# aoschu/esn-ofdm-mimo

Measured on AMD Instinct MI355X. Metric: OFDM symbols/s through the ESN detector (4x8 TDL-B, N=128, N_res=512; train+predict+detect), higher is better.
Workload: dtype f16 operands / f32 accumulate

## Files before the change

### esn_ofdm_mimo_amd/csrc/esn_recur_skew16_impl.h

```cpp
#pragma once
#include "esn_recur_mfma_impl.h"

namespace esn {

constexpr int S16_NKK = 17;
constexpr int S16_NKH = 8;
constexpr int S16_MP = 512;

template <typename TR, int NOISE, bool IO32 = false>
__global__ __launch_bounds__(512) void recur_skew16_kernel(RecurParams p) {
    extern __shared__ __attribute__((aligned(16))) char zf[];
    constexpr int NW = 8, BT = 128, NOWN = 8, NKK = S16_NKK, NKH = S16_NKH;
    constexpr int NTHREADS = NW * 64;
    constexpr int TILE_B = NKK * 1024;
    ESN_STAMP(t_entry)
    const int tid = threadIdx.x;
    const int lane = tid & 63;
    const int wave = __builtin_amdgcn_readfirstlane(tid >> 6);
    const Geometry& g = p.g;
    const int n_res = p.n_res, n_in = p.n_in, n_out = p.n_out;
    const int kin_p = g.kfb - g.kin;
    const int kfb_p = round_up(n_out, 4);
    const int out_rows = p.S - p.transient;

    const int tile = xcd_remap(blockIdx.x, p.n_tiles);
    const int slot0 = tile * BT;
    const int grp0 = slot_group(p, slot0);
    if (grp0 >= p.n_groups) return;
    const int wset = slot_wset(p, slot0);

    int* tab_fr = reinterpret_cast<int*>(zf + (size_t)NOWN * TILE_B);
    uint32_t* tab_key = reinterpret_cast<uint32_t*>(tab_fr + BT);
    float2* tab_in = reinterpret_cast<float2*>(tab_key + BT);
    float2* tab_un = tab_in + NOWN * kin_p;
    char* in_slots = reinterpret_cast<char*>(tab_un + NOWN * 16);
    int* tab_off = reinterpret_cast<int*>(in_slots + (size_t)NOWN * 2048);
    uint32_t* tab_ks = reinterpret_cast<uint32_t*>(tab_off + BT);
    int* tab_grp = reinterpret_cast<int*>(in_slots);
    const int lkin = __builtin_ctz(kin_p);
    for (int i = tid; i < BT; i += NTHREADS) {
        int gtmp;
        const int fr = slot_frame(p, slot0 + i, gtmp);
        tab_fr[i] = fr;
        tab_grp[i] = gtmp;
        tab_key[i] = mix32((uint32_t)p.seed ^ (((uint32_t)fr + p.frame_off) * 0x9E3779B9U));
    }
    {
        constexpr int CHUNKS = NOWN * TILE_B / 16;
        static_assert(CHUNKS % NTHREADS == 0, "whole passes");
#pragma unroll
        for (int i = 0; i < CHUNKS / NTHREADS; ++i)
            *reinterpret_cast<u32x4*>(zf + (size_t)(i * NTHREADS + tid) * 16) = u32x4{0u, 0u, 0u, 0u};
    }
    __syncthreads();
    for (int i = tid; i < NOWN * kin_p; i += NTHREADS) {
        const int c16 = i >> lkin, c = i & (kin_p - 1);
        const int cg = tab_grp[c16 * 16];
        float2 v = make_float2(0.f, 0.f);
        if (cg < p.n_groups && c < n_in) {
            v.x = p.in_scale ? (float)p.in_scale[(size_t)cg * n_in + c] : 1.f;
            v.y = p.in_shift ? (float)p.in_shift[(size_t)cg * n_in + c] : 0.f;
        }
        tab_in[i] = v;
    }
    for (int i = tid; i < NOWN * 16; i += NTHREADS) {
        const int c16 = i / 16, o = i % 16;
        const int cg = tab_grp[c16 * 16];
        float2 v = make_float2(1.f, 0.f);
        if (cg < p.n_groups && o < n_out) {
            if (p.t_scale) v.x = (float)(1.0 / p.t_scale[(size_t)cg * n_out + o]);
            if (p.t_shift) v.y = (float)p.t_shift[(size_t)cg * n_out + o];
        }
        tab_un[i] = v;
    }
#define S16_INLINE __attribute__((always_inline))
    if (p.x0) {
        for (int i = tid; i < BT * 2 * NKH * 4; i += NTHREADS) {
            const int f = i & (BT - 1), kq = i >> 7, kk = kq >> 2, q = kq & 3;
            const bool live = tab_fr[f] >= 0;
            const double* xr = p.x0 + (size_t)(live ? tab_grp[f] : 0) * n_res;
            uint32_t w[4];
#pragma unroll
            for (int t = 0; t < 2; ++t) {
                const int k = 32 * kk + 16 * t + 4 * q;
                float v[4];
#pragma unroll
                for (int e = 0; e < 4; ++e) v[e] = (live && k + e < n_res) ? (float)xr[k + e] : 0.f;
                w[2 * t] = TR::pack2(v[0], v[1]);
                w[2 * t + 1] = TR::pack2(v[2], v[3]);
            }
            *reinterpret_cast<u32x4*>(zf + ((size_t)((f >> 4) * NKK + kk) * 64 + q * 16 + (f & 15)) * 16) = u32x4{w[0], w[1], w[2], w[3]};
        }
    }
    if (p.y0) {
        for (int i = tid; i < BT * 2; i += NTHREADS) {
            const int f = i & (BT - 1), o0 = 4 * (i >> 7);
            const bool live = tab_fr[f] >= 0;
            const double* yr = p.y0 + (size_t)(live ? tab_grp[f] : 0) * n_out;
            float v[4];
#pragma unroll
            for (int e = 0; e < 4; ++e) v[e] = (live && o0 + e < n_out) ? (float)yr[o0 + e] : 0.f;
            const int pos = g.kfb - S16_MP + o0;
            if (o0 < kfb_p)
                TR::store4(zf + ((size_t)((f >> 4) * NKK + 16) * 64 + (pos >> 3) * 16 + (f & 15)) * 16 + 2 * (pos & 7),
                           v[0], v[1], v[2], v[3]);
        }
    }
    __syncthreads();

    const int own_grp = __builtin_amdgcn_readfirstlane(slot_group(p, slot0 + wave * 16));
    const bool has_ro = own_grp < p.n_groups;
    float wo_inv = 1.f;
    if (has_ro)
        wo_inv = *reinterpret_cast<const float*>(reinterpret_cast<const char*>(p.packed_wout)
                                                 + (size_t)own_grp * p.wout_stride + p.wo16_off + (size_t)NKK * 1024);
    const uint32_t in_stride = (uint32_t)(p.T_in * n_in);
    for (int e = tid; e < BT * kin_p; e += NTHREADS) {
        const int f = e >> lkin, ci = e & (kin_p - 1);
        const int fr = tab_fr[f];
        float v = 0.f;
        if (fr >= 0 && ci < n_in) {
            const int row = p.in_row_off;
            const double raw = (row < p.T_in) ? (double)in_ptr<IO32>(p)[(size_t)fr * in_stride + (size_t)row * n_in + ci] : 0.0;
            const float2 ss = tab_in[(f >> 4) * kin_p + ci];
            v = fmaf((float)raw, ss.x, ss.y);
        }
        TR::store1(zf + ((size_t)((f >> 4) * NKK + 16) * 64 + (ci >> 3) * 16 + (f & 15)) * 16 + 2 * (ci & 7), v);
    }

    const float noise = (float)p.noise;
    const float n_c1 = noise * (1.0f / 256.0f), n_c0 = noise * (0.5f / 256.0f - 0.5f);
    f32x4 yacc = {0.f, 0.f, 0.f, 0.f};
    const int lane16 = lane * 16;
    constexpr int OOB = 0x7ffffff0;

    auto finish_readout = [&](int orow, bool write_fb) S16_INLINE {
        int ln_ro = lane;
        asm volatile("" : "+v"(ln_ro));
        const int ofc = ln_ro & 15, oq = ln_ro >> 4;
        if (!has_ro) return;
        const int of = wave * 16 + ofc;
        f32x4 y = yacc;
        const int o0 = 4 * oq;
        const int fr = tab_fr[of];
        const float4* un4 = reinterpret_cast<const float4*>(tab_un + wave * 16 + o0);
        const float4 u01 = un4[0], u23 = un4[1];
#pragma unroll
        for (int j = 0; j < 4; ++j) y[j] += __shfl_xor(y[j], 32);
        y *= wo_inv;
        if (o0 < kfb_p) {
            if (write_fb) {
                const int pos = g.kfb - S16_MP + o0;
                TR::store4(zf + ((size_t)(wave * NKK + 16) * 64 + (pos >> 3) * 16 + ofc) * 16 + 2 * (pos & 7),
                           y[0], y[1], y[2], y[3]);
            }
            if (IO32 && orow >= 0 && fr >= 0) {
                float* yo = p.Y32 + ((size_t)fr * out_rows + orow) * n_out;
                if ((n_out & 3) == 0) {
                    *reinterpret_cast<float4*>(yo + o0) =
                        make_float4((y[0] - u01.y) * u01.x, (y[1] - u01.w) * u01.z, (y[2] - u23.y) * u23.x, (y[3] - u23.w) * u23.z);
                } else {
                    const float2* un = tab_un + wave * 16 + o0;
#pragma unroll
                    for (int j = 0; j < 4; ++j)
                        if (o0 + j < n_out) yo[o0 + j] = (y[j] - un[j].y) * un[j].x;
                }
            } else if (!IO32 && orow >= 0 && fr >= 0) {
                double* yo = p.Y + ((size_t)fr * out_rows + orow) * n_out;
                if ((n_out & 3) == 0) {
                    typedef double f64x2s __attribute__((ext_vector_type(2)));
                    *reinterpret_cast<f64x2s*>(yo + o0) =
                        f64x2s{(double)((y[0] - u01.y) * u01.x), (double)((y[1] - u01.w) * u01.z)};
                    *reinterpret_cast<f64x2s*>(yo + o0 + 2) =
                        f64x2s{(double)((y[2] - u23.y) * u23.x), (double)((y[3] - u23.w) * u23.z)};
                } else {
                    const float2* un = tab_un + wave * 16 + o0;
#pragma unroll
                    for (int j = 0; j < 4; ++j)
                        if (o0 + j < n_out) yo[o0 + j] = (double)((y[j] - un[j].y) * un[j].x);
                }
            }
        }
        yacc = f32x4{0.f, 0.f, 0.f, 0.f};
    };

    const int lag = wave >= NW / 2 ? 1 : 0;
    f32x4 acc[4][8];
    u32x4 abuf[2][4], b[4], ra[4];
    auto zero_acc = [&]() S16_INLINE {
#pragma unroll
        for (int m = 0; m < 4; ++m)
#pragma unroll
            for (int n = 0; n < 8; ++n) acc[m][n] = f32x4{0.f, 0.f, 0.f, 0.f};
    };
    const __amdgpu_buffer_rsrc_t w_rsrc = __builtin_amdgcn_make_buffer_rsrc(
        const_cast<char*>(reinterpret_cast<const char*>(p.packed_w) + (size_t)wset * p.wset_stride + p.w16_off), 0,
        S16_MP * NKK * 64, 0x00020000);
    const int w_frag0 = wave * NKK * 4;
    auto loadA = [&](u32x4 (&a)[4], int kk) S16_INLINE {
        const bool live = kk < NKK;
        const int voff = live ? lane16 : OOB;
#pragma unroll
        for (int m = 0; m < 4; ++m)
            a[m] = __builtin_bit_cast(u32x4, __builtin_amdgcn_raw_buffer_load_b128(
                w_rsrc, voff, live ? (w_frag0 + kk * 4 + m) * 1024 : 0, 0));
    };
    const __amdgpu_buffer_rsrc_t wo_rsrc = __builtin_amdgcn_make_buffer_rsrc(
        const_cast<char*>(reinterpret_cast<const char*>(p.packed_wout)
                          + (size_t)(has_ro ? own_grp : 0) * p.wout_stride + p.wo16_off),
        0, NKK * 1024 + 16, 0x00020000);
    auto load_ra = [&](int j, int kk, bool on) S16_INLINE {
        on = on && kk < 2 * NKH;
        const int voff = on ? lane16 : OOB;
        ra[2 * j] = __builtin_bit_cast(u32x4, __builtin_amdgcn_raw_buffer_load_b128(wo_rsrc, voff, on ? kk * 1024 : 0, 0));
        ra[2 * j + 1] = __builtin_bit_cast(u32x4, __builtin_amdgcn_raw_buffer_load_b128(wo_rsrc, voff, on ? (kk ^ 8) * 1024 : 0, 0));
    };
    auto ro_prefetch = [&](int kk0, bool on) S16_INLINE { load_ra(0, kk0, on); load_ra(1, kk0 + 1, on); };
    typedef const __attribute__((address_space(3))) u32x4* lds_frag_t;
    auto gemm_half = [&](int kk0, auto ro_tag, bool ro_on) S16_INLINE {
        constexpr bool RO = decltype(ro_tag)::value;
        const int voff_ro = ro_on ? lane16 : OOB;
        int ln = lane;
        asm volatile("" : "+v"(ln));
        const uint32_t zb = (uint32_t)(uintptr_t)zf + (uint32_t)(ln << 4);
        uint32_t bp0 = zb + (uint32_t)kk0 * 1024;
        uint32_t bp1 = bp0 + 4 * TILE_B;
#pragma unroll
        for (int n = 0; n < 4; ++n) b[n] = *reinterpret_cast<lds_frag_t>((uintptr_t)(bp0 + n * TILE_B));
        uint32_t rp = zb + (uint32_t)(wave * TILE_B) + (uint32_t)kk0 * 1024;
        uint32_t xp = zb + (uint32_t)(wave * TILE_B) + (uint32_t)(kk0 ^ 8) * 1024;
        int sA = (w_frag0 + (kk0 + 2) * 4) * 1024;
        int sR = (kk0 + 2) * 1024;
        auto trip = [&](int i, auto tail_tag) S16_INLINE {
            constexpr bool TAIL = decltype(tail_tag)::value;
#pragma unroll
            for (int j = 0; j < 2; ++j) {
                const int kk = kk0 + i + j;
                u32x4 rb0, rbx;
#pragma unroll
                for (int n = 0; n < 8; ++n) {
#pragma unroll
                    for (int m = 0; m < 4; ++m) {
                        TR::mma16(acc[m][n], abuf[j][m], b[n & 3]);
                        const int u = n * 4 + m;
                        if (RO) {
                            if (u == 0) rb0 = *reinterpret_cast<lds_frag_t>((uintptr_t)(rp + j * 1024));
                            if (u == 1) rbx = *reinterpret_cast<lds_frag_t>((uintptr_t)(xp + j * 1024));
                            if (u == 8) {
                                TR::mma16(yacc, ra[2 * j], rb0);
                                if (!TAIL)
                                    ra[2 * j] = __builtin_bit_cast(u32x4, __builtin_amdgcn_raw_buffer_load_b128(
                                        wo_rsrc, voff_ro, sR + j * 1024, 0));
                            }
                            if (u == 10) {
                                TR::mma16(yacc, ra[2 * j + 1], rbx);
                                if (!TAIL)
                                    ra[2 * j + 1] = __builtin_bit_cast(u32x4, __builtin_amdgcn_raw_buffer_load_b128(
                                        wo_rsrc, voff_ro, (sR ^ 8192) + j * 1024, 0));
                            }
                        }
                        if (n == 7) {
                            if (TAIL) {
                                const bool live = kk + 2 < NKK;
                                abuf[j][m] = __builtin_bit_cast(u32x4, __builtin_amdgcn_raw_buffer_load_b128(
                                    w_rsrc, live ? lane16 : OOB, live ? (w_frag0 + (kk + 2) * 4 + m) * 1024 : 0, 0));
                            } else {
                                abuf[j][m] = __builtin_bit_cast(u32x4, __builtin_amdgcn_raw_buffer_load_b128(
                                    w_rsrc, lane16, sA + (j * 4 + m) * 1024, 0));
                            }
                        }
                        if (m == 3) {
                            if (n < 4) b[n] = *reinterpret_cast<lds_frag_t>((uintptr_t)(bp1 + n * TILE_B + j * 1024));
                            else b[n - 4] = *reinterpret_cast<lds_frag_t>((uintptr_t)(bp0 + (n - 4) * TILE_B + (j + 1) * 1024));
                        }
                        __builtin_amdgcn_sched_barrier(0);
                    }
                }
            }
            asm volatile("v_add_u32 %0, 2048, %0" : "+v"(bp0));
            asm volatile("v_add_u32 %0, 2048, %0" : "+v"(bp1));
            if (RO) { rp += 2048; xp += 2048; }
            sA += 8192;
            sR += 2048;
        };
        for (int i = 0; i < NKH - 2; i += 2) trip(i, std::false_type{});
        trip(NKH - 2, std::true_type{});
    };
    auto uf_group = [&](u32x4 ra_u) S16_INLINE {
        int ln = lane;
        asm volatile("" : "+v"(ln));
        const uint32_t up = (uint32_t)(uintptr_t)zf + (uint32_t)(ln << 4) + 16 * 1024;
#pragma unroll
        for (int n = 0; n < 4; ++n) b[n] = *reinterpret_cast<lds_frag_t>((uintptr_t)(up + n * TILE_B));
        {
            const u32x4 rb_u = *reinterpret_cast<lds_frag_t>((uintptr_t)(up + wave * TILE_B));
            TR::mma16(yacc, ra_u, rb_u);
        }
#pragma unroll
        for (int n = 0; n < 8; ++n) {
#pragma unroll
            for (int m = 0; m < 4; ++m) TR::mma16(acc[m][n], abuf[0][m], b[n & 3]);
            if (n < 4) b[n] = *reinterpret_cast<lds_frag_t>((uintptr_t)(up + (n + 4) * TILE_B));
            __builtin_amdgcn_sched_barrier(0);
        }
    };
    auto next_step_A = [&]() S16_INLINE { loadA(abuf[0], 0); loadA(abuf[1], 1); };

    constexpr bool PK_NOISE = NOISE == ESN_NOISE_COUNTER && std::is_same<TR, TraitsF16>::value;
    typedef _Float16 h16x2 __attribute__((ext_vector_type(2)));
    typedef float f32x2 __attribute__((ext_vector_type(2)));
    const _Float16 c1s = (_Float16)(1024.0f * n_c1);
    const h16x2 c1h = {c1s, c1s};
    const float t_bias = 1.0f + n_c0 - (float)c1s;
    const uint32_t seed_hi = (uint32_t)(p.seed >> 32);
    auto activate = [&](int s, auto n0_tag, auto n1_tag, int ln) S16_INLINE {
        constexpr int N0 = decltype(n0_tag)::value, N1 = decltype(n1_tag)::value;
        const int g4 = ln >> 4, col = ln & 15;
        uint32_t k1[N1 - N0];
        int frs[N1 - N0];
#pragma unroll
        for (int n = N0; n < N1; ++n) {
            const int t = n;
            if (NOISE == ESN_NOISE_COUNTER) k1[n - N0] = tab_ks[(s & 1) * BT + t * 16 + col];
            if (NOISE == ESN_NOISE_TENSOR) frs[n - N0] = tab_fr[t * 16 + col];
        }
#pragma unroll
        for (int n = N0; n < N1; ++n) {
            const int t = n;
            uint32_t key = 0;
            const double* nz = nullptr;
            if (NOISE == ESN_NOISE_COUNTER)
                key = k1[n - N0] + (uint32_t)(16 * wave + g4) * 0x9E3779B9U;
            if (NOISE == ESN_NOISE_TENSOR && frs[n - N0] >= 0)
                nz = p.noise_u + ((size_t)frs[n - N0] * p.S + s) * n_res;
            char* dst = zf + (size_t)t * TILE_B + (size_t)(2 * wave) * 1024 + (size_t)ln * 16;
#pragma unroll
            for (int pr = 0; pr < 2; ++pr) {
                uint32_t out[4];
#pragma unroll
                for (int tt = 0; tt < 2; ++tt) {
                    const int m = 2 * pr + tt;
                    const f32x4 a4 = acc[m][n];
                    if constexpr (PK_NOISE) {
                        float tv[4];
#pragma unroll
                        for (int j = 0; j < 4; ++j) {
                            const float e = __builtin_amdgcn_exp2f(a4[j]);
                            tv[j] = fmaf(-2.0f, __builtin_amdgcn_rcpf(e + 1.0f), t_bias);
                        }
                        const uint32_t sq = noise_mix(key + (uint32_t)(4 * m) * 0x9E3779B9U);
                        const h16x2 w01 = __builtin_bit_cast(h16x2, __builtin_amdgcn_perm(0x3C3C3C3Cu, sq, 0x04010400u));
                        const h16x2 w23 = __builtin_bit_cast(h16x2, __builtin_amdgcn_perm(0x3C3C3C3Cu, sq, 0x04030402u));
                        const h16x2 t01 = __builtin_convertvector(f32x2{tv[0], tv[1]}, h16x2);
                        const h16x2 t23 = __builtin_convertvector(f32x2{tv[2], tv[3]}, h16x2);
                        out[2 * tt] = __builtin_bit_cast(uint32_t, __builtin_elementwise_fma(w01, c1h, t01));
                        out[2 * tt + 1] = __builtin_bit_cast(uint32_t, __builtin_elementwise_fma(w23, c1h, t23));
                    } else {
                        float v[4];
#pragma unroll
                        for (int j = 0; j < 4; ++j) v[j] = TR::act(a4[j]);
                        const int row = 64 * wave + 16 * m + 4 * g4;
                        if (NOISE == ESN_NOISE_COUNTER) {
                            const uint32_t sq = noise_mix(key + (uint32_t)(4 * m) * 0x9E3779B9U);
                            v[0] = fmaf((float)(sq & 0xffU), n_c1, v[0] + n_c0);
                            v[1] = fmaf((float)((sq >> 8) & 0xffU), n_c1, v[1] + n_c0);
                            v[2] = fmaf((float)((sq >> 16) & 0xffU), n_c1, v[2] + n_c0);
                            v[3] = fmaf((float)(sq >> 24), n_c1, v[3] + n_c0);
                        } else if (NOISE == ESN_NOISE_TENSOR) {
#pragma unroll
                            for (int j = 0; j < 4; ++j) {
                                const bool on = nz && row + j < n_res;
                                const double u = (on ? nz : p.noise_u)[on ? row + j : 0];
                                const float w = v[j] + noise * ((float)u - 0.5f);
                                v[j] = on ? w : v[j];
                            }
                        }
                        out[2 * tt] = TR::pack2(v[0], v[1]);
                        out[2 * tt + 1] = TR::pack2(v[2], v[3]);
                    }
                }
                *reinterpret_cast<u32x4*>(dst + pr * 1024) = u32x4{out[0], out[1], out[2], out[3]};
                __builtin_amdgcn_sched_barrier(0);
            }
        }
    };
    const std::integral_constant<int, 0> n_lo;
    const std::integral_constant<int, 4> n_mid;
    const std::integral_constant<int, 8> n_hi;

    const bool in_w16 = !IO32 || (n_in & 3) == 0;
    const int cpf = IO32 ? (in_w16 ? n_in / 4 : n_in) : n_in / 2;
    constexpr int IN_TRIPS = IO32 ? 1 : 2;
    constexpr int IN_TILES = NOWN / (NW / 2);
    const int in_c0 = IN_TILES * (wave - NW / 2);
    const int lcpf = __builtin_ctz(cpf);
    const size_t in_frame_bytes = (size_t)in_stride * sizeof(io_elem<IO32>);
    int j0;
    slot_group(p, slot0, j0);
    size_t u_base_frame = j0 < p.F ? (size_t)grp0 * p.F + j0 : ((size_t)grp0 + (p.spw ? p.n_wsets : 1)) * p.F;
    if (u_base_frame >= (size_t)p.n_frames) u_base_frame = (size_t)p.n_frames - 1;
    for (int i = tid; i < BT; i += NTHREADS) {
        const int fr = tab_fr[i];
        tab_off[i] = fr >= 0 ? (int)(((size_t)fr - u_base_frame) * in_frame_bytes) : -1;
    }
    __syncthreads();
    const size_t u_left = ((size_t)p.n_frames - u_base_frame) * in_frame_bytes;
    const uintptr_t u_base = reinterpret_cast<uintptr_t>(p.U) + u_base_frame * in_frame_bytes;
    const uint32_t u_base_lo = __builtin_amdgcn_readfirstlane((uint32_t)u_base);
    const uint32_t u_base_hi = __builtin_amdgcn_readfirstlane((uint32_t)(u_base >> 32));
    const int u_records = __builtin_amdgcn_readfirstlane((int)(u_left < 0x7fffffffu ? u_left : 0x7fffffffu));
    const __amdgpu_buffer_rsrc_t u_rsrc = __builtin_amdgcn_make_buffer_rsrc(
        reinterpret_cast<char*>(((uintptr_t)u_base_hi << 32) | u_base_lo), 0, u_records, 0x00020000);
    auto dma_inputs_b = [&](int s) S16_INLINE {
        const int row = s + p.in_row_off;
        const bool row_ok = row < p.T_in;
        int ln = lane;
        asm volatile("" : "+v"(ln));
        int off[IN_TILES][IN_TRIPS];
#pragma unroll
        for (int ti = 0; ti < IN_TILES; ++ti)
#pragma unroll
            for (int i = 0; i < IN_TRIPS; ++i) {
                const int e = 64 * i + ln;
                off[ti][i] = tab_off[(in_c0 + ti) * 16 + ((e >> lcpf) & 15)];
            }
#pragma unroll
        for (int ti = 0; ti < IN_TILES; ++ti) {
            const int c = in_c0 + ti;
#pragma unroll
            for (int i = 0; i < IN_TRIPS; ++i) {
                const int e = 64 * i + ln;
                const bool on = off[ti][i] >= 0 && row_ok && e < 16 * cpf;
                if constexpr (IO32) {
                    auto* slot = (__attribute__((address_space(3))) void*)(in_slots + (size_t)(c * 2 + i) * 1024);
                    const int voff = on ? off[ti][i] + ((e & (cpf - 1)) << (in_w16 ? 4 : 2)) : OOB;
                    if (in_w16)
                        __builtin_amdgcn_raw_ptr_buffer_load_lds(u_rsrc, slot, 16, voff, row_ok ? row * n_in * 4 : 0, 0, 0);
                    else
                        __builtin_amdgcn_raw_ptr_buffer_load_lds(u_rsrc, slot, 4, voff, row_ok ? row * n_in * 4 : 0, 0, 0);
                } else {
                    const int voff = on ? off[ti][i] + ((e & (cpf - 1)) << 4) : OOB;
                    __builtin_amdgcn_raw_ptr_buffer_load_lds(
                        u_rsrc, (__attribute__((address_space(3))) void*)(in_slots + (size_t)(c * 2 + i) * 1024), 16,
                        voff, row_ok ? row * n_in * 8 : 0, 0, 0);
                }
            }
        }
    };
    auto commit_inputs_b = [&](int s) S16_INLINE {
        const bool row_ok = s + p.in_row_off < p.T_in;
        const int lk2 = lkin - 1;
        int ln = lane;
        asm volatile("" : "+v"(ln));
#pragma unroll
        for (int ti = 0; ti < IN_TILES; ++ti) {
            const int c = in_c0 + ti;
#pragma unroll
            for (int k = 0; k < 2; ++k) {
                const int e2 = ln + 64 * k;
                const int f = (e2 >> lk2) & 15, c2 = e2 & ((kin_p >> 1) - 1), ci = 2 * c2;
                const bool live = tab_fr[c * 16 + f] >= 0 && ci < n_in;
                const float4 ss = *reinterpret_cast<const float4*>(tab_in + c * kin_p + ci);
                double2 raw;
                if constexpr (IO32) {
                    const float2 r32 = *reinterpret_cast<const float2*>(in_slots + (size_t)c * 2048 + (size_t)(f * n_in + ci) * 4);
                    raw = double2{(double)r32.x, (double)r32.y};
                } else {
                    const int ch = (f << lcpf) + c2;
                    raw = *reinterpret_cast<const double2*>(
                        in_slots + (size_t)(c * 2 + (ch >> 6)) * 1024 + (size_t)(ch & 63) * 16);
                }
                const float v0 = live ? fmaf((float)(row_ok ? raw.x : 0.0), ss.x, ss.y) : 0.f;
                const float v1 = live ? fmaf((float)(row_ok ? raw.y : 0.0), ss.z, ss.w) : 0.f;
                if (e2 < 8 * kin_p)
                    TR::store2(zf + ((size_t)(c * NKK + 16) * 64 + (ci >> 3) * 16 + f) * 16 + 2 * (ci & 7), v0, v1);
                __builtin_amdgcn_sched_barrier(0);
            }
        }
    };

#ifdef ESN_STAMPS
    unsigned long long sk_acc[14] = {0, 0, 0, 0, 0, 0, 0, 0, 0, 0, 0, 0, 0, 0};
#define ESN_SK_ADD(i, a, b) sk_acc[i] += (b) - (a);
#define ESN_SYNC_SPLIT(mid) __builtin_amdgcn_fence(__ATOMIC_RELEASE, "workgroup"); ESN_STAMP(mid) \
    __builtin_amdgcn_s_barrier(); __builtin_amdgcn_fence(__ATOMIC_ACQUIRE, "workgroup");
#else
#define ESN_SK_ADD(i, a, b)
#define ESN_SYNC_SPLIT(mid) __syncthreads();
#endif
    const uint32_t key1_own = tab_key[wave * 16 + (lane & 15)];
    ESN_STAMP(t_prologue)
    auto run_set = [&](auto lag_tag) S16_INLINE {
        constexpr bool LAG = decltype(lag_tag)::value;
        next_step_A();
        if (LAG) {
            ro_prefetch(0, false);
            __syncthreads();
        }
        for (int s = 0; s < p.S; ++s) {
            const bool ro = has_ro && s > 0;
            ESN_STAMP(t0)
            zero_acc();
            if (LAG) __builtin_amdgcn_s_setprio(1);
            if (NOISE == ESN_NOISE_COUNTER) {
                const uint32_t k = mix32(key1_own ^ seed_hi ^ ((uint32_t)s * 0x85EBCA6BU + 0x27d4eb2fU));
                if (lane < 16) tab_ks[(s & 1) * BT + wave * 16 + lane] = k;
            }
            if (LAG) {
                if (s > 0) commit_inputs_b(s);
                gemm_half(0, std::true_type{}, ro);
                if (ro) finish_readout(s - 1 - p.transient, true);
                __builtin_amdgcn_s_setprio(0);
            } else {
                gemm_half(0, std::false_type{}, false);
                ro_prefetch(NKH, ro);
            }
            ESN_STAMP(t1)
            ESN_SYNC_SPLIT(m1)
            ESN_STAMP(t2)
#ifdef ESN_STAMPS
            unsigned long long u3 = 0, u4 = 0;
#endif
            auto load_ra_u = [&]() S16_INLINE {
                return __builtin_bit_cast(u32x4, __builtin_amdgcn_raw_buffer_load_b128(
                    wo_rsrc, has_ro ? lane16 : OOB, has_ro ? 16 * 1024 : 0, 0));
            };
            u32x4 ra_u;
            if (LAG) {
                gemm_half(NKH, std::false_type{}, false);
                ra_u = load_ra_u();
                ESN_STAMP_SET(u3)
                if (s + 1 < p.S) dma_inputs_b(s + 1);
                ESN_STAMP_SET(u4)
            } else {
                gemm_half(NKH, std::true_type{}, ro);
                if (ro) finish_readout(s - 1 - p.transient, true);
                ra_u = load_ra_u();
            }
            ESN_STAMP(t3)
            ESN_SYNC_SPLIT(m3)
            ESN_STAMP(t4)
            __builtin_amdgcn_s_setprio(2);
            int ln_e = lane;
            asm volatile("" : "+v"(ln_e));
            uf_group(ra_u);
            ESN_STAMP(u1)
            activate(s, n_lo, n_mid, ln_e);
            ESN_STAMP(u2)
            next_step_A();
            if (LAG) ro_prefetch(0, has_ro && s + 1 < p.S);
            ESN_STAMP(u2b)
            activate(s, n_mid, n_hi, ln_e);
            ESN_STAMP(u5)
            __builtin_amdgcn_s_setprio(0);
            ESN_STAMP(t5)
            __syncthreads();
            ESN_STAMP(t6)
            ESN_SK_ADD(0, t0, t1) ESN_SK_ADD(1, t1, t2) ESN_SK_ADD(2, t2, t3)
            ESN_SK_ADD(3, t3, t4) ESN_SK_ADD(4, t4, t5) ESN_SK_ADD(5, t5, t6)
            ESN_SK_ADD(6, t4, u1) ESN_SK_ADD(7, u1, u2) ESN_SK_ADD(8, u2, u2b) ESN_SK_ADD(9, u3, u4)
            ESN_SK_ADD(10, u2b, u5) ESN_SK_ADD(11, u5, t5) ESN_SK_ADD(12, t1, m1) ESN_SK_ADD(13, t3, m3)
        }
    };
    if (lag) run_set(std::true_type{}); else run_set(std::false_type{});
#undef ESN_SK_ADD
#undef ESN_SYNC_SPLIT
#ifdef ESN_STAMPS
    if (p.stamps && blockIdx.x == 0 && lane == 0) {
        p.stamps[wave * 8 + 7] = t_prologue - t_entry;
        for (int i = 0; i < 2; ++i) p.stamps[(8 + wave) * 8 + 6 + i] = sk_acc[12 + i];
        for (int i = 0; i < 6; ++i) p.stamps[wave * 8 + i] = sk_acc[i];
        for (int i = 0; i < 6; ++i) p.stamps[(8 + wave) * 8 + i] = sk_acc[6 + i];
        p.stamps[wave * 8 + 6] = (unsigned long long)__builtin_amdgcn_s_getreg(63492);
    }
#endif
    if (!lag) __syncthreads();
    if (has_ro) {
        for (int kk = 0; kk < 2 * NKH; ++kk) {
            const u32x4 rb = *reinterpret_cast<const u32x4*>(zf + (size_t)(wave * NKK + kk) * 1024 + lane16);
            const u32x4 rw = __builtin_bit_cast(u32x4, __builtin_amdgcn_raw_buffer_load_b128(wo_rsrc, lane16, kk * 1024, 0));
            TR::mma16(yacc, rw, rb);
        }
        finish_readout(p.S - 1 - p.transient, false);
    }
}
#undef S16_INLINE

template <typename TR, bool IO32>
static int launch_skew16(const RecurParams& p, hipStream_t stream) {
    const int kin_p = p.g.kfb - p.g.kin;
    const size_t lds = (size_t)8 * S16_NKK * 1024 + 4 * 128 + 4 * 128 + 8 * (size_t)8 * (kin_p + 16) + 8 * 2048 + 4 * 128 + 8 * 128;
    auto go = [&](auto kern) -> int {
        hipError_t e = hipFuncSetAttribute(reinterpret_cast<const void*>(kern), hipFuncAttributeMaxDynamicSharedMemorySize, (int)lds);
        if (e != hipSuccess) return (int)e;
        hipLaunchKernelGGL(kern, dim3(p.n_tiles), dim3(512), lds, stream, p);
        return (int)hipGetLastError();
    };
    switch (p.noise_mode) {
        case ESN_NOISE_NONE: return go(recur_skew16_kernel<TR, ESN_NOISE_NONE, IO32>);
        case ESN_NOISE_TENSOR: return go(recur_skew16_kernel<TR, ESN_NOISE_TENSOR, IO32>);
        default: return go(recur_skew16_kernel<TR, ESN_NOISE_COUNTER, IO32>);
    }
}

}
```

Measured before the change: 11.92 million.

## Split input commit into load/store and reissue DMA at step start

Moves the per-step input commit and next-step DMA launch to the top of each LAG step. The commit is split into an LDS-read phase and a store phase, with the asynchronous buffer-to-LDS load for step s+1 issued between them. Static LDS now holds the image and tables, and only the input slots stay in dynamic shared memory. The initial input fill loop is dropped in favour of a DMA for step 0. Barriers in the LAG path become raw lgkmcnt waits plus s_barrier, and a vmcnt(0) wait is added before activation. This risks correctness if waits are missing, and the static LDS size hardcodes kin_p=16.

```diff
diff --git a/esn_ofdm_mimo_amd/csrc/esn_recur_skew16_impl.h b/esn_ofdm_mimo_amd/csrc/esn_recur_skew16_impl.h
--- a/esn_ofdm_mimo_amd/csrc/esn_recur_skew16_impl.h
+++ b/esn_ofdm_mimo_amd/csrc/esn_recur_skew16_impl.h
@@ -6,10 +6,12 @@
 constexpr int S16_NKK = 17;
 constexpr int S16_NKH = 8;
 constexpr int S16_MP = 512;
+constexpr int S16_IMAGE_LDS = 8 * S16_NKK * 1024 + 4 * 128 + 4 * 128 + 8 * 8 * (16 + 16) + 4 * 128 + 8 * 128;
 
 template <typename TR, int NOISE, bool IO32 = false>
 __global__ __launch_bounds__(512) void recur_skew16_kernel(RecurParams p) {
-    extern __shared__ __attribute__((aligned(16))) char zf[];
+    __shared__ __attribute__((aligned(16))) char zf[S16_IMAGE_LDS];
+    extern __shared__ __attribute__((aligned(16))) char in_slots[];
     constexpr int NW = 8, BT = 128, NOWN = 8, NKK = S16_NKK, NKH = S16_NKH;
     constexpr int NTHREADS = NW * 64;
     constexpr int TILE_B = NKK * 1024;
@@ -33,8 +35,7 @@
     uint32_t* tab_key = reinterpret_cast<uint32_t*>(tab_fr + BT);
     float2* tab_in = reinterpret_cast<float2*>(tab_key + BT);
     float2* tab_un = tab_in + NOWN * kin_p;
-    char* in_slots = reinterpret_cast<char*>(tab_un + NOWN * 16);
-    int* tab_off = reinterpret_cast<int*>(in_slots + (size_t)NOWN * 2048);
+    int* tab_off = reinterpret_cast<int*>(tab_un + NOWN * 16);
     uint32_t* tab_ks = reinterpret_cast<uint32_t*>(tab_off + BT);
     int* tab_grp = reinterpret_cast<int*>(in_slots);
     const int lkin = __builtin_ctz(kin_p);
@@ -115,19 +116,6 @@
         wo_inv = *reinterpret_cast<const float*>(reinterpret_cast<const char*>(p.packed_wout)
                                                  + (size_t)own_grp * p.wout_stride + p.wo16_off + (size_t)NKK * 1024);
     const uint32_t in_stride = (uint32_t)(p.T_in * n_in);
-    for (int e = tid; e < BT * kin_p; e += NTHREADS) {
-        const int f = e >> lkin, ci = e & (kin_p - 1);
-        const int fr = tab_fr[f];
-        float v = 0.f;
-        if (fr >= 0 && ci < n_in) {
-            const int row = p.in_row_off;
-            const double raw = (row < p.T_in) ? (double)in_ptr<IO32>(p)[(size_t)fr * in_stride + (size_t)row * n_in + ci] : 0.0;
-            const float2 ss = tab_in[(f >> 4) * kin_p + ci];
-            v = fmaf((float)raw, ss.x, ss.y);
-        }
-        TR::store1(zf + ((size_t)((f >> 4) * NKK + 16) * 64 + (ci >> 3) * 16 + (f & 15)) * 16 + 2 * (ci & 7), v);
-    }
-
     const float noise = (float)p.noise;
     const float n_c1 = noise * (1.0f / 256.0f), n_c0 = noise * (0.5f / 256.0f - 0.5f);
     f32x4 yacc = {0.f, 0.f, 0.f, 0.f};
@@ -411,19 +399,22 @@
     const int u_records = __builtin_amdgcn_readfirstlane((int)(u_left < 0x7fffffffu ? u_left : 0x7fffffffu));
     const __amdgpu_buffer_rsrc_t u_rsrc = __builtin_amdgcn_make_buffer_rsrc(
         reinterpret_cast<char*>(((uintptr_t)u_base_hi << 32) | u_base_lo), 0, u_records, 0x00020000);
-    auto dma_inputs_b = [&](int s) S16_INLINE {
+    auto dma_offsets_b = [&](int (&off)[IN_TILES][IN_TRIPS]) S16_INLINE {
+        int ln = lane;
+        asm volatile("" : "+v"(ln));
+#pragma unroll
+        for (int ti = 0; ti < IN_TILES; ++ti)
+#pragma unroll
+            for (int i = 0; i < IN_TRIPS; ++i) {
+                const int e = 64 * i + ln;
+                off[ti][i] = tab_off[(in_c0 + ti) * 16 + ((e >> lcpf) & 15)];
+            }
+    };
+    auto dma_launch_b = [&](int s, const int (&off)[IN_TILES][IN_TRIPS]) S16_INLINE {
         const int row = s + p.in_row_off;
         const bool row_ok = row < p.T_in;
         int ln = lane;
         asm volatile("" : "+v"(ln));
-        int off[IN_TILES][IN_TRIPS];
-#pragma unroll
-        for (int ti = 0; ti < IN_TILES; ++ti)
-#pragma unroll
-            for (int i = 0; i < IN_TRIPS; ++i) {
-                const int e = 64 * i + ln;
-                off[ti][i] = tab_off[(in_c0 + ti) * 16 + ((e >> lcpf) & 15)];
-            }
 #pragma unroll
         for (int ti = 0; ti < IN_TILES; ++ti) {
             const int c = in_c0 + ti;
@@ -447,7 +438,36 @@
             }
         }
     };
-    auto commit_inputs_b = [&](int s) S16_INLINE {
+    struct CommitRegs {
+        int fr[IN_TILES][2];
+        float4 ss[IN_TILES][2];
+        double2 raw[IN_TILES][2];
+    };
+    auto commit_load_b = [&](CommitRegs& r) S16_INLINE {
+        const int lk2 = lkin - 1;
+        int ln = lane;
+        asm volatile("" : "+v"(ln));
+#pragma unroll
+        for (int ti = 0; ti < IN_TILES; ++ti) {
+            const int c = in_c0 + ti;
+#pragma unroll
+            for (int k = 0; k < 2; ++k) {
+                const int e2 = ln + 64 * k;
+                const int f = (e2 >> lk2) & 15, c2 = e2 & ((kin_p >> 1) - 1), ci = 2 * c2;
+                r.fr[ti][k] = tab_fr[c * 16 + f];
+                r.ss[ti][k] = *reinterpret_cast<const float4*>(tab_in + c * kin_p + ci);
+                if constexpr (IO32) {
+                    const float2 r32 = *reinterpret_cast<const float2*>(in_slots + (size_t)c * 2048 + (size_t)(f * n_in + ci) * 4);
+                    r.raw[ti][k] = double2{(double)r32.x, (double)r32.y};
+                } else {
+                    const int ch = (f << lcpf) + c2;
+                    r.raw[ti][k] = *reinterpret_cast<const double2*>(
+                        in_slots + (size_t)(c * 2 + (ch >> 6)) * 1024 + (size_t)(ch & 63) * 16);
+                }
+            }
+        }
+    };
+    auto commit_store_b = [&](int s, const CommitRegs& r) S16_INLINE {
         const bool row_ok = s + p.in_row_off < p.T_in;
         const int lk2 = lkin - 1;
         int ln = lane;
@@ -459,22 +479,10 @@
             for (int k = 0; k < 2; ++k) {
                 const int e2 = ln + 64 * k;
                 const int f = (e2 >> lk2) & 15, c2 = e2 & ((kin_p >> 1) - 1), ci = 2 * c2;
-                const bool live = tab_fr[c * 16 + f] >= 0 && ci < n_in;
-                const float4 ss = *reinterpret_cast<const float4*>(tab_in + c * kin_p + ci);
-                double2 raw;
-                if constexpr (IO32) {
-                    const float2 r32 = *reinterpret_cast<const float2*>(in_slots + (size_t)c * 2048 + (size_t)(f * n_in + ci) * 4);
-                    raw = double2{(double)r32.x, (double)r32.y};
-                } else {
-                    const int ch = (f << lcpf) + c2;
-                    raw = *reinterpret_cast<const double2*>(
-                        in_slots + (size_t)(c * 2 + (ch >> 6)) * 1024 + (size_t)(ch & 63) * 16);
-                }
-                const float v0 = live ? fmaf((float)(row_ok ? raw.x : 0.0), ss.x, ss.y) : 0.f;
-                const float v1 = live ? fmaf((float)(row_ok ? raw.y : 0.0), ss.z, ss.w) : 0.f;
-                if (e2 < 8 * kin_p)
-                    TR::store2(zf + ((size_t)(c * NKK + 16) * 64 + (ci >> 3) * 16 + f) * 16 + 2 * (ci & 7), v0, v1);
-                __builtin_amdgcn_sched_barrier(0);
+                const bool live = (r.fr[ti][k] >= 0) & (ci < n_in);
+                const float v0 = live ? fmaf((float)(row_ok ? r.raw[ti][k].x : 0.0), r.ss[ti][k].x, r.ss[ti][k].y) : 0.f;
+                const float v1 = live ? fmaf((float)(row_ok ? r.raw[ti][k].y : 0.0), r.ss[ti][k].z, r.ss[ti][k].w) : 0.f;
+                TR::store2(zf + ((size_t)(c * NKK + 16) * 64 + (ci >> 3) * 16 + f) * 16 + 2 * (ci & 7), v0, v1);
             }
         }
     };
@@ -482,32 +490,56 @@
 #ifdef ESN_STAMPS
     unsigned long long sk_acc[14] = {0, 0, 0, 0, 0, 0, 0, 0, 0, 0, 0, 0, 0, 0};
 #define ESN_SK_ADD(i, a, b) sk_acc[i] += (b) - (a);
-#define ESN_SYNC_SPLIT(mid) __builtin_amdgcn_fence(__ATOMIC_RELEASE, "workgroup"); ESN_STAMP(mid) \
-    __builtin_amdgcn_s_barrier(); __builtin_amdgcn_fence(__ATOMIC_ACQUIRE, "workgroup");
+#define ESN_SYNC_SPLIT(mid) unsigned long long mid; if (LAG) { asm volatile("s_waitcnt lgkmcnt(0)" ::: "memory"); \
+    ESN_STAMP_SET(mid) asm volatile("s_barrier" ::: "memory"); } else { __builtin_amdgcn_fence(__ATOMIC_RELEASE, "workgroup"); \
+    ESN_STAMP_SET(mid) __builtin_amdgcn_s_barrier(); __builtin_amdgcn_fence(__ATOMIC_ACQUIRE, "workgroup"); }
 #else
 #define ESN_SK_ADD(i, a, b)
-#define ESN_SYNC_SPLIT(mid) __syncthreads();
+#define ESN_SYNC_SPLIT(mid) sync_set();
 #endif
-    const uint32_t key1_own = tab_key[wave * 16 + (lane & 15)];
     ESN_STAMP(t_prologue)
     auto run_set = [&](auto lag_tag) S16_INLINE {
         constexpr bool LAG = decltype(lag_tag)::value;
+        auto sync_set = [&]() S16_INLINE {
+            if (LAG) asm volatile("s_waitcnt lgkmcnt(0)\n\ts_barrier" ::: "memory");
+            else __syncthreads();
+        };
         next_step_A();
         if (LAG) {
+            {
+                int off[IN_TILES][IN_TRIPS];
+                dma_offsets_b(off);
+                dma_launch_b(0, off);
+            }
             ro_prefetch(0, false);
             __syncthreads();
         }
         for (int s = 0; s < p.S; ++s) {
             const bool ro = has_ro && s > 0;
             ESN_STAMP(t0)
+#ifdef ESN_STAMPS
+            unsigned long long u3 = 0, u4 = 0;
+#endif
+            if (LAG) {
+                __builtin_amdgcn_s_setprio(1);
+                ESN_STAMP_SET(u3)
+                CommitRegs cr;
+                int off[IN_TILES][IN_TRIPS];
+                dma_offsets_b(off);
+                commit_load_b(cr);
+                asm volatile("s_waitcnt lgkmcnt(0)" ::: "memory");
+                if (s + 1 < p.S) dma_launch_b(s + 1, off);
+                commit_store_b(s, cr);
+                ESN_STAMP_SET(u4)
+            }
             zero_acc();
-            if (LAG) __builtin_amdgcn_s_setprio(1);
             if (NOISE == ESN_NOISE_COUNTER) {
-                const uint32_t k = mix32(key1_own ^ seed_hi ^ ((uint32_t)s * 0x85EBCA6BU + 0x27d4eb2fU));
-                if (lane < 16) tab_ks[(s & 1) * BT + wave * 16 + lane] = k;
+                int ln_k = lane;
+                asm volatile("" : "+v"(ln_k));
+                const uint32_t k = mix32(tab_key[wave * 16 + (ln_k & 15)] ^ seed_hi ^ ((uint32_t)s * 0x85EBCA6BU + 0x27d4eb2fU));
+                tab_ks[(s & 1) * BT + wave * 16 + (ln_k & 15)] = k;
             }
             if (LAG) {
-                if (s > 0) commit_inputs_b(s);
                 gemm_half(0, std::true_type{}, ro);
                 if (ro) finish_readout(s - 1 - p.transient, true);
                 __builtin_amdgcn_s_setprio(0);
@@ -518,9 +550,6 @@
             ESN_STAMP(t1)
             ESN_SYNC_SPLIT(m1)
             ESN_STAMP(t2)
-#ifdef ESN_STAMPS
-            unsigned long long u3 = 0, u4 = 0;
-#endif
             auto load_ra_u = [&]() S16_INLINE {
                 return __builtin_bit_cast(u32x4, __builtin_amdgcn_raw_buffer_load_b128(
                     wo_rsrc, has_ro ? lane16 : OOB, has_ro ? 16 * 1024 : 0, 0));
@@ -529,9 +558,6 @@
             if (LAG) {
                 gemm_half(NKH, std::false_type{}, false);
                 ra_u = load_ra_u();
-                ESN_STAMP_SET(u3)
-                if (s + 1 < p.S) dma_inputs_b(s + 1);
-                ESN_STAMP_SET(u4)
             } else {
                 gemm_half(NKH, std::true_type{}, ro);
                 if (ro) finish_readout(s - 1 - p.transient, true);
@@ -544,6 +570,7 @@
             int ln_e = lane;
             asm volatile("" : "+v"(ln_e));
             uf_group(ra_u);
+            if (LAG) asm volatile("s_waitcnt vmcnt(0)" ::: "memory");
             ESN_STAMP(u1)
             activate(s, n_lo, n_mid, ln_e);
             ESN_STAMP(u2)
@@ -554,7 +581,7 @@
             ESN_STAMP(u5)
             __builtin_amdgcn_s_setprio(0);
             ESN_STAMP(t5)
-            __syncthreads();
+            sync_set();
             ESN_STAMP(t6)
             ESN_SK_ADD(0, t0, t1) ESN_SK_ADD(1, t1, t2) ESN_SK_ADD(2, t2, t3)
             ESN_SK_ADD(3, t3, t4) ESN_SK_ADD(4, t4, t5) ESN_SK_ADD(5, t5, t6)
@@ -588,8 +615,7 @@
 
 template <typename TR, bool IO32>
 static int launch_skew16(const RecurParams& p, hipStream_t stream) {
-    const int kin_p = p.g.kfb - p.g.kin;
-    const size_t lds = (size_t)8 * S16_NKK * 1024 + 4 * 128 + 4 * 128 + 8 * (size_t)8 * (kin_p + 16) + 8 * 2048 + 4 * 128 + 8 * 128;
+    const size_t lds = 8 * 2048;
     auto go = [&](auto kern) -> int {
         hipError_t e = hipFuncSetAttribute(reinterpret_cast<const void*>(kern), hipFuncAttributeMaxDynamicSharedMemorySize, (int)lds);
         if (e != hipSuccess) return (int)e;
```

New measurement: 11.74 million. -1.5%, worse.
